# Changfei-Fu/RUMI-SLAM

Hardware: AMD Instinct MI355X
Metric: frames/sec ORB extract+match (higher is better)
Workload: dtype u8; 1 GPU; ORB extract (640x480, 8-level pyramid, 1000 features/frame) + brute-force 256-bit Hamming match of consecutive frames (BASELINE.json configs[1]+[2]); scaling=n/a (one GPU), exchange=none

## Files before the change

include/rumi_testhooks.h:

```cpp
#ifndef RUMI_TESTHOOKS_H
#define RUMI_TESTHOOKS_H
#include <stdint.h>
#ifdef __cplusplus
extern "C" {
#endif

int rumi_hook_sort_like_std(uint32_t *keys, uint16_t *ids, int32_t n);
int rumi_hook_sort_device(uint32_t *keys, uint16_t *ids, int32_t n);
int rumi_hook_std_sort(uint32_t *keys, uint16_t *ids, int32_t n);

int rumi_hook_quadtree(const uint32_t *cand, int32_t n, int32_t minX, int32_t maxX, int32_t minY, int32_t maxY,
                       int32_t N, int32_t *out_idx, int32_t cap, int32_t *n_out);

float rumi_hook_sinf(float x);
float rumi_hook_cosf(float x);
float rumi_hook_fast_atan2(float y, float x);
int rumi_hook_cv_round(float v);
int rumi_hook_magic_div(int32_t idx, int32_t d);

int rumi_hook_lane_packing(int32_t w, int32_t h, float scale, int32_t nlevels, int32_t nframes, int32_t kernel, int32_t level, int32_t force_g,
                           int32_t *info, int32_t *slots, int32_t cap, int32_t *n_out);

struct RumiMatcher;
int rumi_hook_newpts_matches(struct RumiMatcher *m, int32_t n_neigh, int32_t n1, int32_t *matches);

#ifdef __cplusplus
}
#endif
#endif
```

rumi_slam_amd/capi.py:

```python
import ctypes as C
import os

import numpy as np

_HERE = os.path.dirname(os.path.abspath(__file__))
LIB_PATH = os.path.join(_HERE, "librumi_hip.so")

RUMI_OK, RUMI_E_INVALID, RUMI_E_NO_DEVICE, RUMI_E_CAPACITY, RUMI_E_EMPTY = 0, -1, -2, -3, -4

KP_DTYPE = np.dtype([("x", "<f4"), ("y", "<f4"), ("size", "<f4"), ("angle", "<f4"),
                     ("response", "<f4"), ("octave", "<i4"), ("class_id", "<i4")])
assert KP_DTYPE.itemsize == 28


class RumiOrbConfig(C.Structure):
    _fields_ = [("nfeatures", C.c_int32), ("scale_factor", C.c_float), ("nlevels", C.c_int32),
                ("ini_th_fast", C.c_int32), ("min_th_fast", C.c_int32), ("max_width", C.c_int32),
                ("max_height", C.c_int32), ("max_batch", C.c_int32), ("device", C.c_int32),
                ("host_threads", C.c_int32), ("blur_variant", C.c_int32)]


class RumiStreamFrame(C.Structure):
    _fields_ = [("n", C.c_int32), ("mono", C.c_int32), ("n_prev", C.c_int32), ("kp", C.c_void_p), ("desc", C.c_void_p),
                ("best_idx", C.c_void_p), ("best_dist", C.c_void_p), ("second_dist", C.c_void_p)]
# ... 40 lines not shown
    L.rumi_orb_extract_batch_device_async.argtypes = L.rumi_orb_extract_batch_device.argtypes
    L.rumi_orb_sync.argtypes = [vp]
    L.rumi_orb_extract_batch_records_async.argtypes = [vp, vp, i32, i32, i32, i32, i64, i32, i32, vp, i64, i32, vp]
    L.rumi_orb_extract_batch_host.argtypes = [vp, vp, i32, i32, i32, i32, i32, i32, vp, vp, vp, i32, vp, vp, vp, vp]
    L.rumi_orb_extract_batch_host_records.argtypes = [vp, vp, i32, i32, i32, i32, i32, i32, vp, i64, i32, vp, vp]
    L.rumi_orb_pyramid_level.argtypes = [vp, i32, i32, i32, i32, vp, i32, C.POINTER(i32), C.POINTER(i32)]
    L.rumi_orb_stage_keypoints.argtypes = [vp, i32, i32, i32, vp, i32, C.POINTER(i32)]
    L.rumi_orb_set_profiling.argtypes = [vp, i32]
    L.rumi_orb_set_resident_queue.argtypes = [vp, i32]
    L.rumi_orb_wait_event.argtypes = [vp, vp]
    L.rumi_orb_stage_ms.argtypes = [vp, vp]
    L.rumi_orb_stream_create.argtypes = [vp, C.POINTER(vp)]
    L.rumi_orb_stream_destroy.argtypes = [vp]
    L.rumi_orb_stream_destroy.restype = None
    L.rumi_orb_stream_reset.argtypes = [vp]
    L.rumi_orb_stream_push.argtypes = [vp, vp, i32, i32, i32, i32, i32, C.POINTER(RumiStreamFrame)]
    L.rumi_orb_stream_resident.argtypes = [vp, C.POINTER(vp), C.POINTER(vp), C.POINTER(vp)]
    _lib = L
    return L


def check(code):
    if code != RUMI_OK:
        raise RumiError(code, lib().rumi_last_error().decode("utf-8", "replace"))


def ptr(a):
    return a.ctypes.data_as(C.c_void_p)


MATCH_SYMBOLS = ["rumi_descriptor_distance", "rumi_match_create", "rumi_match_destroy", "rumi_search_by_projection_mappoints",
                 "rumi_search_by_projection_frame", "rumi_search_by_bow", "rumi_search_by_bow_kf", "rumi_search_by_projection_sim3",
                 "rumi_search_by_projection_reloc", "rumi_search_for_initialization", "rumi_search_for_triangulation", "rumi_fuse_candidates", "rumi_search_by_sim3", "rumi_frame_is_in_frustum", "rumi_search_local_points", "rumi_search_by_bow_batch", "rumi_match_bruteforce_batch_device", "rumi_match_bruteforce_batch_device_strided", "rumi_match_bruteforce_ring_device", "rumi_match_bruteforce_shape", "rumi_submap_match",
                 "rumi_match_bruteforce_pair_scratch_bytes", "rumi_match_bruteforce_pair_shape", "rumi_match_bruteforce_pair_device"]

OPT_SYMBOLS = ["rumi_opt_create", "rumi_opt_destroy", "rumi_pose_optimization", "rumi_pose_optimization_batch", "rumi_local_ba", "rumi_local_ba_batch", "rumi_merge_ba", "rumi_bundle_adjustment", "rumi_sim3_inliers",
               "rumi_optimize_sim3", "rumi_sim3_ransac", "rumi_opt_stage_ms", "rumi_opt_set_profiling", "rumi_opt_kernel_ms",
               "rumi_essential_graph", "rumi_sim3_correct_points"]

VOC_SYMBOLS = ["rumi_voc_create", "rumi_voc_load_text", "rumi_voc_destroy", "rumi_voc_words", "rumi_voc_levels", "rumi_voc_set_levels", "rumi_voc_assemble", "rumi_voc_transform_features",
               "rumi_voc_transform_batch_device", "rumi_voc_transform"]
TRACK_SYMBOLS = ["rumi_track_create", "rumi_track_destroy", "rumi_track_frame", "rumi_track_extract", "rumi_track_motion",
                 "rumi_track_reference_keyframe", "rumi_track_local", "rumi_track_image_buffer", "rumi_track_last_projections", "rumi_track_set_distortion", "rumi_track_undistorted"]
QUEUE_SYMBOLS = ["rumi_queue_create", "rumi_queue_destroy", "rumi_queue_shards", "rumi_queue_record_bytes", "rumi_queue_block_capacity", "rumi_queue_row",
                 "rumi_queue_uses_rccl", "rumi_queue_extract", "rumi_queue_last_ms"]
KFDB_SYMBOLS = ["rumi_kfdb_create", "rumi_kfdb_destroy", "rumi_kfdb_clear", "rumi_kfdb_size", "rumi_kfdb_next_seq", "rumi_kfdb_max_batch", "rumi_kfdb_add",
                "rumi_kfdb_add_batch_device", "rumi_kfdb_bow", "rumi_kfdb_erase", "rumi_kfdb_clear_map", "rumi_kfdb_set_map_bad", "rumi_kfdb_set_maps",
                "rumi_kfdb_set_bad", "rumi_kfdb_set_covisibles", "rumi_kfdb_score", "rumi_kfdb_scored", "rumi_kfdb_select_reloc", "rumi_kfdb_select_nbest"]
MAPPING_SYMBOLS = ["rumi_create_new_map_points", "rumi_refresh_create", "rumi_refresh_destroy", "rumi_refresh_map_points", "rumi_refresh_stage_ms",
                   "rumi_cull_create", "rumi_cull_destroy", "rumi_keyframe_culling", "rumi_cull_stage_ms"]


def kfdb_lib():
    L = lib()
    if getattr(L, "_kfdb_ready", False):
        return L
    vp, i32, i64, u64 = C.c_void_p, C.c_int32, C.c_int64, C.c_uint64
    L.rumi_kfdb_create.argtypes = [vp, i32, i64, i32, C.POINTER(vp)]
    L.rumi_kfdb_destroy.argtypes = [vp]
    L.rumi_kfdb_destroy.restype = None
    L.rumi_kfdb_clear.argtypes = [vp]
    L.rumi_kfdb_size.argtypes = [vp]
    L.rumi_kfdb_next_seq.argtypes = [vp]
    L.rumi_kfdb_next_seq.restype = i64
    L.rumi_kfdb_max_batch.argtypes = [vp]
    L.rumi_kfdb_add.argtypes = [vp, i32, vp, vp, vp, vp, vp]
    L.rumi_kfdb_add_batch_device.argtypes = [vp, i32, vp, vp, vp, vp, vp, i32, vp]
    L.rumi_kfdb_bow.argtypes = [vp, u64, vp, vp, i32, C.POINTER(i32)]
    L.rumi_kfdb_erase.argtypes = [vp, i32, vp]
    L.rumi_kfdb_clear_map.argtypes = [vp, i32]
    L.rumi_kfdb_set_map_bad.argtypes = [vp, i32, i32]
    L.rumi_kfdb_set_maps.argtypes = [vp, i32, vp, vp]
    L.rumi_kfdb_set_bad.argtypes = [vp, i32, vp, vp]
    L.rumi_kfdb_set_covisibles.argtypes = [vp, i32, vp, vp]
    L.rumi_kfdb_score.argtypes = [vp, i32, i32, vp, vp, vp, vp, vp, vp, vp, vp, vp]
    L.rumi_kfdb_scored.argtypes = [vp, vp, vp]
    L.rumi_kfdb_select_reloc.argtypes = [vp, vp, vp, i64]
    L.rumi_kfdb_select_nbest.argtypes = [vp, vp, i32, vp, vp, vp, vp]
    L._kfdb_ready = True
    return L


HOOK_SYMBOLS = ["rumi_hook_sort_like_std", "rumi_hook_sort_device", "rumi_hook_std_sort", "rumi_hook_quadtree", "rumi_hook_sinf", "rumi_hook_cosf",
                "rumi_hook_fast_atan2", "rumi_hook_cv_round", "rumi_hook_magic_div", "rumi_hook_newpts_matches", "rumi_hook_lane_packing"]


def hooks():
    L = lib()
    if getattr(L, "_hooks_ready", False):
        return L
    vp, i32 = C.c_void_p, C.c_int32
    L.rumi_hook_sort_like_std.argtypes = [vp, vp, i32]
    L.rumi_hook_sort_device.argtypes = [vp, vp, i32]
    L.rumi_hook_std_sort.argtypes = [vp, vp, i32]
    L.rumi_hook_quadtree.argtypes = [vp, i32, i32, i32, i32, i32, i32, vp, i32, C.POINTER(i32)]
    for name in ("rumi_hook_sinf", "rumi_hook_cosf"):
        getattr(L, name).restype = C.c_float
        getattr(L, name).argtypes = [C.c_float]
    L.rumi_hook_fast_atan2.restype = C.c_float
    L.rumi_hook_fast_atan2.argtypes = [C.c_float, C.c_float]
    L.rumi_hook_cv_round.argtypes = [C.c_float]
    L.rumi_hook_magic_div.argtypes = [i32, i32]
    L.rumi_hook_lane_packing.argtypes = [i32, i32, C.c_float, i32, i32, i32, i32, i32, vp, vp, i32, C.POINTER(i32)]
    L._hooks_ready = True
    return L
```

rumi_slam_amd/csrc/orb_kernels.hip:

```cpp
#include <hip/hip_runtime.h>

#include "orb_device.h"
#include "orb_math.h"

namespace rumi {

struct PatternF { float v[256 * 4]; };
constexpr PatternF make_pattern_f() {
    constexpr int8_t src[256 * 4] = {
#include "orb_pattern.inc"
    };
    PatternF p{};
    for (int i = 0; i < 256 * 4; i++) p.v[i] = (float)src[i];
    return p;
}
__constant__ PatternF c_patternF = make_pattern_f();

__device__ __forceinline__ unsigned xcd_swizzle(unsigned lin, unsigned total) {
    const unsigned q = total >> 3, r = total & 7, xcd = lin & 7;
    return (xcd < r ? xcd * (q + 1) : r * (q + 1) + (xcd - r) * q) + (lin >> 3);
}

struct __attribute__((packed)) U32 { uint32_t v; };
struct __attribute__((packed)) U64 { uint64_t v; };
// ... 744 lines not shown
        C = *reinterpret_cast<const uint32_t *>(row);
        H = 0;
        if (!kPacked && haloOff) H = *reinterpret_cast<const uint32_t *>(row + haloOff);
    };
#pragma unroll
    for (int j = 0; j < 7; j++) fetch(y0 - 3 + j, Cn[j], Hn[j]);
    uint32_t Cm[7], Hm[7];
    auto walk7 = [&](const uint32_t (&Cc)[7], const uint32_t (&Hc)[7], int r0) {
#pragma unroll
        for (int j = 0; j < 7; j++) {
            const int r = r0 + j;
            if (r >= rEnd) break;
            orow += L.pitch;
            uint32_t C = Cc[j];
            if (edgeWave) {
                const uint32_t c1 = __shfl_up(C, 1), c2 = __shfl_up(c1, 1);
                C = __builtin_amdgcn_perm(C, __builtin_amdgcn_perm(c1, c2, selA), selB);
            }
            uint32_t Lw = __shfl_up(C, 1), Rw = __shfl_down(C, 1);
            if constexpr (kPacked) {
                if (seamWave && first) Lw = __builtin_amdgcn_perm(C, C, 0x01020300u);
            } else {
                if (lane == 0) Lw = firstBlock ? __builtin_amdgcn_perm(C, C, 0x01020300u) : Hc[j];
                if (lane == 63 && !edgeWave && bw == 256) Rw = Hc[j];
            }
            constexpr uint32_t tA = 18u | (34u << 8) | (kT2 << 16) | (kT3 << 24), tB = kT2 | (34u << 8) | (18u << 16);
            const uint32_t A0 = __builtin_amdgcn_alignbyte(C, Lw, 1), A1 = __builtin_amdgcn_alignbyte(C, Lw, 2), A2 = __builtin_amdgcn_alignbyte(C, Lw, 3);
            const uint32_t B0 = __builtin_amdgcn_alignbyte(Rw, C, 1), B1 = __builtin_amdgcn_alignbyte(Rw, C, 2), B2 = __builtin_amdgcn_alignbyte(Rw, C, 3);
            ring[j][0] = (int)__builtin_amdgcn_udot4(B0, tB, __builtin_amdgcn_udot4(A0, tA, 0u, false), false);
            ring[j][1] = (int)__builtin_amdgcn_udot4(B1, tB, __builtin_amdgcn_udot4(A1, tA, 0u, false), false);
            ring[j][2] = (int)__builtin_amdgcn_udot4(B2, tB, __builtin_amdgcn_udot4(A2, tA, 0u, false), false);
            ring[j][3] = (int)__builtin_amdgcn_udot4(Rw, tB, __builtin_amdgcn_udot4(C, tA, 0u, false), false);
            const int y = r - 3;
            if (y >= y0 && produce) {
                uint32_t o[4];
#pragma unroll
                for (int i = 0; i < 4; i++) {
                    uint32_t acc = mad_u24(kT3, (uint32_t)ring[(j + 4) % 7][i], 32768u);
                    acc = mad_u24(kT2, (uint32_t)(ring[(j + 3) % 7][i] + ring[(j + 5) % 7][i]), acc);
                    acc = mad_u24(34u, (uint32_t)(ring[(j + 2) % 7][i] + ring[(j + 6) % 7][i]), acc);
                    acc = mad_u24(18u, (uint32_t)(ring[(j + 1) % 7][i] + ring[j][i]), acc);
                    if (VARIANT) acc = min(acc, 0x00FFFFFFu);
                    o[i] = acc;
                }
                const uint32_t p01 = __builtin_amdgcn_perm(o[1], o[0], 0x0c0c0602u), p23 = __builtin_amdgcn_perm(o[3], o[2], 0x06020c0cu);
                *reinterpret_cast<uint32_t *>(orow) = p01 | p23;
            }
        }
    };
    for (int r0 = y0 - 3; r0 < rEnd; r0 += 7) {
#pragma unroll
        for (int j = 0; j < 7; j++) Cm[j] = Cn[j], Hm[j] = Hn[j];
        if (r0 + 7 < rEnd) {
#pragma unroll
            for (int j = 0; j < 7; j++) fetch(r0 + 7 + j, Cn[j], Hn[j]);
        }
        walk7(Cm, Hm, r0);
    }
}
template <int VARIANT, int kBlurRows>
__global__ __launch_bounds__(256) void k_blur(const DevParams *__restrict__ P, ImgSrc src, BlurGrid G) {
    blur_body<VARIANT, kBlurRows, false>(P, src, G, blockIdx.x, gridDim.x);
}
template <int VARIANT>
__global__ __launch_bounds__(256) void k_blur_packed(const DevParams *__restrict__ P, ImgSrc src, BlurPack G) {
    blur_body<VARIANT, kBlurRowsBatch, true>(P, src, G, blockIdx.x, gridDim.x);
}
template <int TPC, int VARIANT>
__global__ __launch_bounds__(256) void k_fast_blur(const DevParams *__restrict__ P, ImgSrc src, FastLds F, uint32_t *__restrict__ cellBuf,
                                                   int32_t *__restrict__ cellCnt, BlurGrid G, unsigned gxFast) {
    if (blockIdx.x < gxFast) fast_cells_body<TPC>(P, src, F, cellBuf, cellCnt, blockIdx.x, gxFast);
    else blur_body<VARIANT, kBlurRowsSmall, false>(P, src, G, blockIdx.x - gxFast, gridDim.x - gxFast);
}

__device__ __forceinline__ int half_wave_sum(int v) {
    v += __builtin_amdgcn_update_dpp(0, v, 0x111, 0xF, 0xF, false);
    v += __builtin_amdgcn_update_dpp(0, v, 0x112, 0xF, 0xF, false);
    v += __builtin_amdgcn_update_dpp(0, v, 0x114, 0xF, 0xF, false);
    v += __builtin_amdgcn_update_dpp(0, v, 0x118, 0xF, 0xF, false);
    v += __builtin_amdgcn_update_dpp(0, v, 0x142, 0xA, 0xF, false);
    const int lo = __builtin_amdgcn_readlane(v, 31), hi = __builtin_amdgcn_readlane(v, 63);
    return (threadIdx.x & 32) ? hi : lo;
}
__device__ __forceinline__ int wave_sum(int v) {
#pragma unroll
    for (int o = 32; o > 0; o >>= 1) v += __shfl_xor(v, o);
    return v;
}

constexpr int kDiscP = 48, kPatchP = 48;
constexpr int kKpPerWg = 8;

struct AssembleArgs {
    const uint32_t *selLevel; const int32_t *selLevelCnt; int selLevelCap, lap0, lap1;
    int32_t *counts; long long countsStride; int32_t *errFlag, *errMirror;
    uint32_t *selPackedOut, *selMetaOut; int32_t *selCountOut;
};
template <int kKpGroups, bool kAssemble>
__global__ __launch_bounds__(256, 7) void k_orient_desc(const DevParams *__restrict__ P, ImgSrc src,
                                                     const uint32_t *__restrict__ selPacked,
                                                     const uint32_t *__restrict__ selMeta,
                                                     const int32_t *__restrict__ selCount, int selCap,
                                                     RumiKeyPoint *__restrict__ kpOut, long long kpStride, uint8_t *__restrict__ descOut,
                                                     long long descStride, int outCap, AssembleArgs A) {
    static_assert(kDiscP == kPatchP, "the disc and the patch share their rows");
    __shared__ __attribute__((aligned(16))) uint8_t sWin[kKpPerWg][37 * kPatchP];
    __shared__ __attribute__((aligned(16))) float sPat[256 * 4];
    __shared__ int4 sLv[kMaxLevels];
    __shared__ float2 sLvF[kMaxLevels];
    reinterpret_cast<float4 *>(sPat)[threadIdx.x] = reinterpret_cast<const float4 *>(c_patternF.v)[threadIdx.x];
    if (threadIdx.x < (unsigned)P->nlevels) {
        const DevLevel &Lv = P->lv[threadIdx.x];
        sLv[threadIdx.x] = threadIdx.x == 0 ? make_int4(0, src.l0Pitch, (int)Lv.off, Lv.pitch) : make_int4((int)Lv.off, Lv.pitch, (int)Lv.off, Lv.pitch);
        sLvF[threadIdx.x] = make_float2(Lv.scale, Lv.patchSize);
    }
    const int lane = threadIdx.x & 31, hw = threadIdx.x >> 5;
    const unsigned wg = xcd_swizzle(blockIdx.y * gridDim.x + blockIdx.x, gridDim.x * gridDim.y);
    const int kb = (wg % gridDim.x) * (kKpPerWg * kKpGroups) + hw, frame = wg / gridDim.x;
    int cnt;
    __shared__ uint32_t sOwnPk[kAssemble ? kKpPerWg * kKpGroups : 1], sOwnMt[kAssemble ? kKpPerWg * kKpGroups : 1];
    if constexpr (!kAssemble) {
        cnt = selCount[frame];
        __syncthreads();
    } else {
        __shared__ int sLvStart[kMaxLevels + 1], sRed[2], sOwnF[kKpPerWg * kKpGroups];
        const int nl = P->nlevels, tid = threadIdx.x;
        if (tid == 0) {
            int run = 0;
            for (int l = 0; l < nl; l++) { sLvStart[l] = run; run += A.selLevelCnt[(long long)frame * nl + l]; }
            sLvStart[nl] = run; sRed[0] = 0; sRed[1] = 0;
        }
        __syncthreads();
        const int total = sLvStart[nl], kbase = (wg % gridDim.x) * (kKpPerWg * kKpGroups);
        const bool first = wg % gridDim.x == 0, over = total > selCap;
        int32_t *counts = reinterpret_cast<int32_t *>(reinterpret_cast<uint8_t *>(A.counts) + frame * A.countsStride);
        if (over) {
            if (first && tid == 0) { A.selCountOut[frame] = 0; counts[0] = total; counts[1] = 0; const int old = atomicOr(A.errFlag, 8); if (A.errMirror) *A.errMirror = old | 8; }
            return;
        }
        cnt = total;
        auto key_at = [&](int k, int *levelOut) -> uint32_t {
            int level = 0;
            while (k >= sLvStart[level + 1]) level++;
            *levelOut = level;
            return A.selLevel[((long long)frame * nl + level) * A.selLevelCap + (k - sLvStart[level])];
        };
        auto lapped = [&](uint32_t pk, int level) -> bool {
            float x = (float)((int)(pk & 0xFFF) + kBorder);
            if (level != 0) x = x * P->lv[level].scale;
            return x >= (float)A.lap0 && x <= (float)A.lap1;
        };
        int before = 0, all = 0;
        for (int k = tid; k < total; k += 256) {
            int level;
            const uint32_t pk = key_at(k, &level);
            const int f = lapped(pk, level) ? 1 : 0;
            all += f; before += k < kbase ? f : 0;
        }
#pragma unroll
        for (int o = 32; o > 0; o >>= 1) { before += __shfl_xor(before, o); all += __shfl_xor(all, o); }
        if ((tid & 63) == 0) { atomicAdd(&sRed[0], before); atomicAdd(&sRed[1], all); }
        if (tid < kKpPerWg * kKpGroups) {
            const int k = kbase + tid;
            int level = 0;
            uint32_t pk = 0;
            int f = 0;
            if (k < total) { pk = key_at(k, &level); f = lapped(pk, level) ? 1 : 0; }
            sOwnPk[tid] = pk; sOwnMt[tid] = (uint32_t)level; sOwnF[tid] = f;
        }
        __syncthreads();
        if (tid == 0) {
            int b = sRed[0];
            for (int j = 0; j < kKpPerWg * kKpGroups; j++) {
                const int k = kbase + j;
                if (k >= total) break;
                const int f = sOwnF[j], slot = f ? (total - 1 - b) : (k - b);
                b += f;
                sOwnMt[j] |= (uint32_t)slot << 8;
            }
            if (first) {
                counts[0] = total; counts[1] = total - sRed[1];
                A.selCountOut[frame] = total;
                if (A.errMirror) *A.errMirror = *A.errFlag;
            }
        }
        __syncthreads();
        if (tid < kKpPerWg * kKpGroups && kbase + tid < total) {
            A.selPackedOut[(long long)frame * selCap + kbase + tid] = sOwnPk[tid];
            A.selMetaOut[(long long)frame * selCap + kbase + tid] = sOwnMt[tid];
        }
    }
#ifdef RUMI_OD_STAMP
    long long st[8] = {0, 0, 0, 0, 0, 0, 0, 0}, stLast = clock64();
#define OD_STAMP(k) do { const long long t_ = clock64(); st[k] += t_ - stLast; stLast = t_; } while (0)
#else
#define OD_STAMP(k) do { } while (0)
#endif

    struct __attribute__((packed, aligned(4))) Q16 { uint32_t x, y, z, w; };
    struct __attribute__((packed, aligned(4))) Q8 { uint32_t x, y; };
    auto ld16 = [](const uint8_t *q) { const Q16 t = *reinterpret_cast<const Q16 *>(q); return make_uint4(t.x, t.y, t.z, t.w); };
    auto ld8 = [](const uint8_t *q) { const Q8 t = *reinterpret_cast<const Q8 *>(q); return make_uint2(t.x, t.y); };
    struct Staged { uint4 d0, d1, p0, p1, q0, q1; uint2 p2, q2; uint32_t d2; };
    const bool dRow = lane < 31, qRow = lane < 5;
    const uint8_t *frame0 = src.l0 + (long long)frame * src.l0FrameStride, *framePyr = src.pyr + (long long)frame * P->arenaStride,
                  *frameBlur = src.blur + (long long)frame * P->arenaStride;
    auto fetch_disc = [&](uint32_t pk, uint32_t meta, bool live, Staged &S) {
        if (!live || !dRow) return;
        const int level = meta & 0xFF, x = (int)(pk & 0xFFF) + kBorder, y = (int)((pk >> 12) & 0xFFF) + kBorder;
        const int4 lv = sLv[level];
        const uint8_t *cr = (level == 0 ? frame0 : framePyr) + (lv.x + (y - kHalfPatch + lane) * lv.y + ((x - kHalfPatch) & ~3));
        S.d0 = ld16(cr); S.d1 = ld16(cr + 16); S.d2 = *reinterpret_cast<const uint32_t *>(cr + 32);
    };
    auto fetch_patch = [&](uint32_t pk, uint32_t meta, bool live, Staged &S) {
        if (!live) return;
        const int level = meta & 0xFF, x = (int)(pk & 0xFFF) + kBorder, y = (int)((pk >> 12) & 0xFFF) + kBorder;
        const int4 lv = sLv[level];
        const uint8_t *br = frameBlur + (lv.z + (y - 18 + lane) * lv.w + ((x - 18) & ~3)), *br2 = br + 32 * lv.w;
        S.p0 = ld16(br); S.p1 = ld16(br + 16); S.p2 = ld8(br + 32);
        if (qRow) { S.q0 = ld16(br2); S.q1 = ld16(br2 + 16); S.q2 = ld8(br2 + 32); }
    };
    auto stage_disc = [&](bool live, const Staged &S) {
        if (!live || !dRow) return;
        uint8_t *dst = &sWin[hw][lane * kDiscP];
        *reinterpret_cast<uint4 *>(dst) = S.d0; *reinterpret_cast<uint4 *>(dst + 16) = S.d1; *reinterpret_cast<uint32_t *>(dst + 32) = S.d2;
    };
    auto stage_patch = [&](bool live, const Staged &S) {
        if (!live) return;
        {
            uint8_t *dst = &sWin[hw][lane * kPatchP];
            *reinterpret_cast<uint4 *>(dst) = S.p0; *reinterpret_cast<uint4 *>(dst + 16) = S.p1; *reinterpret_cast<uint2 *>(dst + 32) = S.p2;
        }
        if (qRow) {
            uint8_t *dst = &sWin[hw][(lane + 32) * kPatchP];
            *reinterpret_cast<uint4 *>(dst) = S.q0; *reinterpret_cast<uint4 *>(dst + 16) = S.q1; *reinterpret_cast<uint2 *>(dst + 32) = S.q2;
        }
    };
    auto orientation = [&](uint32_t pk) -> float {
        const int x = (int)(pk & 0xFFF) + kBorder;
        const int xd = (x - kHalfPatch) & ~3;
        const uint8_t *dc = &sWin[hw][kHalfPatch * kDiscP + (x - xd)];
        const int u = lane - kHalfPatch;
        const int vmaxU = lane < 31 ? P->umax[u < 0 ? -u : u] : -1;
        const int mid = dc[u];
        int colSum = vmaxU >= 0 ? mid : 0, m01 = 0;
#pragma unroll
        for (int v = 1; v <= kHalfPatch; v++) {
            const int lo = dc[-v * kDiscP + u], hi = dc[v * kDiscP + u];
            const bool in = v <= vmaxU;
            colSum += in ? lo + hi : 0;
            m01 += in ? v * (hi - lo) : 0;
        }
        int m10 = u * colSum;
        m10 = half_wave_sum(m10);
        m01 = half_wave_sum(m01);
        OD_STAMP(4);
        return fast_atan2_deg((float)m01, (float)m10);
    };
    auto describe = [&](uint32_t pk, uint32_t meta, float angle) {
        const int level = meta & 0xFF, slot = (int)(meta >> 8);
        const int x = (int)(pk & 0xFFF) + kBorder, y = (int)((pk >> 12) & 0xFFF) + kBorder, score = (int)(pk >> 24);
        const int xp = (x - 18) & ~3;
        const float factorPI = (float)(3.1415926535897932384626433832795 / 180.f);
        const float ang = angle * factorPI;
        const float a = cosf_glibc(ang), b = sinf_glibc(ang);
        const uint8_t *bc = &sWin[hw][18 * kPatchP + (x - xp)];
        uint32_t w = 0;
        OD_STAMP(5);
#pragma unroll
        for (int j = 0; j < 8; j++) {
            const float4 pt = reinterpret_cast<const float4 *>(sPat)[j * 32 + lane];
            const float x0 = pt.x, y0 = pt.y, x1 = pt.z, y1 = pt.w;
            const int r0 = cv_round_f(x0 * b + y0 * a), c0 = cv_round_f(x0 * a - y0 * b);
            const int r1 = cv_round_f(x1 * b + y1 * a), c1 = cv_round_f(x1 * a - y1 * b);
            const int t0 = bc[r0 * kPatchP + c0], t1 = bc[r1 * kPatchP + c1];
            const unsigned long long bal = __ballot(t0 < t1);
            const uint32_t lo = (uint32_t)bal, hi = (uint32_t)(bal >> 32);
            asm("s_nop 4\n\tv_writelane_b32 %0, %1, %3\n\tv_writelane_b32 %0, %2, %4" : "+v"(w) : "s"(lo), "s"(hi), "n"(j), "n"(32 + j));
        }
        OD_STAMP(6);
        if (slot < outCap) {
            if (lane < 8) reinterpret_cast<uint32_t *>(descOut + frame * descStride + (long long)slot * 32)[lane] = w;
            if (lane == 0) {
                RumiKeyPoint kp;
                kp.x = (float)x; kp.y = (float)y;
                const float2 lf = sLvF[level];
                if (level != 0) { kp.x = kp.x * lf.x; kp.y = kp.y * lf.x; }
                kp.size = lf.y;
                kp.angle = angle;
                kp.response = (float)score;
                kp.octave = level;
                kp.class_id = -1;
                reinterpret_cast<RumiKeyPoint *>(reinterpret_cast<uint8_t *>(kpOut) + frame * kpStride)[slot] = kp;
            }
        }
    };

    const uint32_t *selP = selPacked + (long long)frame * selCap, *selM = selMeta + (long long)frame * selCap;
    auto key_rec = [&](int k, uint32_t &pk, uint32_t &mt) {
        if constexpr (kAssemble) { const int j = k - (kb - hw); pk = sOwnPk[j]; mt = sOwnMt[j]; }
        else { pk = selP[k]; mt = selM[k]; }
    };
    bool liveC = kb < cnt, liveN = kb + kKpPerWg < cnt;
    uint32_t pkC = 0, mtC = 0, pkN = 0, mtN = 0;
    if (liveC) key_rec(kb, pkC, mtC);
    if (liveN && kKpGroups > 1) key_rec(kb + kKpPerWg, pkN, mtN);
    if (kKpGroups == 1) liveN = false;
    Staged S;
    fetch_disc(pkC, mtC, liveC, S);
    fetch_patch(pkC, mtC, liveC, S);
#pragma unroll
    for (int g = 0; g < kKpGroups; g++) {
        if (!__any(liveC)) break;
        OD_STAMP(0);
        stage_disc(liveC, S);
        OD_STAMP(1);
        const int k2 = kb + (g + 2) * kKpPerWg;
        const bool liveNN = g + 2 < kKpGroups && k2 < cnt;
        uint32_t pkNN = 0, mtNN = 0;
        if (liveNN) key_rec(k2, pkNN, mtNN);
        if (g + 1 < kKpGroups) fetch_disc(pkN, mtN, liveN, S);
        OD_STAMP(2);
        float angle = 0.f;
        if (liveC) angle = orientation(pkC);
        stage_patch(liveC, S);
        if (g + 1 < kKpGroups) fetch_patch(pkN, mtN, liveN, S);
        if (liveC) describe(pkC, mtC, angle);
        OD_STAMP(3);
        pkC = pkN; mtC = mtN; liveC = liveN;
        pkN = pkNN; mtN = mtNN; liveN = liveNN;
    }
#ifdef RUMI_OD_STAMP
    if (threadIdx.x == 0 && (blockIdx.x % 8) == 0 && blockIdx.y == 0) printf("od wg %d: loop-head %lld stage(wait loads) %lld issue-next %lld | IC_Angle %lld trig %lld rBRIEF %lld store %lld\n", (int)blockIdx.x, st[0], st[1], st[2], st[4], st[5], st[6], st[3]);
#endif
}

static long long pack_span(const DevParams &hP, const ImgSrc &src, bool readsLevel0) {
    if (readsLevel0 && src.l0FrameStride <= 0) return 0;
    return readsLevel0 ? std::max(hP.arenaStride, src.l0FrameStride) : hP.arenaStride;
}
void launch_resize(const DevParams *dP, const DevParams &hP, ImgSrc src, const int16_t *coef, const RowTap *rowTab, int level, int nframes,
                   hipStream_t st, int32_t *clearWord) {
    const int rows = hP.lv[level].h >= 200 ? 8 : 4;
    const LanePack K = resize_pack_of(hP.lv[level].w, nframes, pack_span(hP, src, level == 1));
    dim3 g(K.waves, (hP.lv[level].h + 4 * rows - 1) / (4 * rows), (nframes + K.G - 1) / K.G);
    if (rows == 8) hipLaunchKernelGGL(k_resize<8>, g, dim3(256), 0, st, dP, src, coef, rowTab, level, clearWord, K, nframes);
    else hipLaunchKernelGGL(k_resize<4>, g, dim3(256), 0, st, dP, src, coef, rowTab, level, clearWord, K, nframes);
}
void launch_pyramid_tiles(const DevParams *dP, ImgSrc src, const int16_t *coef, const RowTap *rowTab, const PyrTile *tiles, int ntiles, int bufBytes,
                          int tabEntries, int nframes, hipStream_t st, int32_t *clearWord) {
    hipLaunchKernelGGL(k_pyramid_tiles, dim3(ntiles, nframes), dim3(256), (size_t)2 * bufBytes + (size_t)tabEntries * 8, st, dP, src, coef, rowTab, tiles, bufBytes, clearWord);
}
static FastLds fast_lds_of(const DevParams &hP) {
    int wMax = 0, hMax = 0;
    for (int l = 0; l < hP.nlevels; l++) { wMax = std::max(wMax, hP.lv[l].wCell); hMax = std::max(hMax, hP.lv[l].hCell); }
    FastLds F;
    F.tp = 4 * (((wMax + 3) >> 2) + 2);
    F.sp = F.tp;
    F.tileBytes = (hMax + 6) * F.tp;
    F.scBytes = ((hMax + 2) * F.sp + 15) & ~15;
    F.maxIters = (wMax * hMax + 63) / 64 + 1;
    F.tileBytes = (F.tileBytes + 15) & ~15;
    F.perWave = (F.tileBytes + F.scBytes + std::max(kRingCap * 2, F.maxIters * 8) + kScoredCap * 2 + 15) & ~15;
    return F;
}
void launch_fast(const DevParams *dP, const DevParams &hP, ImgSrc src, uint32_t *cellBuf, int32_t *cellCnt, int nframes,
                 hipStream_t st) {
    const FastLds F = fast_lds_of(hP);
    const int wpg = 4;
    const dim3 grid((hP.totalCells + wpg - 1) / wpg, nframes);
    const size_t lds = (size_t)wpg * F.perWave;
#define RUMI_FAST_CASE(T)                                                                                      \
    if (F.tp == T) {                                                                                           \
        hipLaunchKernelGGL((k_fast_cells<T>), grid, dim3(64 * wpg), lds, st, dP, src, F, cellBuf, cellCnt);    \
        return;                                                                                                \
    }
    RUMI_FAST_CASE(48) RUMI_FAST_CASE(44) RUMI_FAST_CASE(52) RUMI_FAST_CASE(56)
#undef RUMI_FAST_CASE
    hipLaunchKernelGGL((k_fast_cells<0>), grid, dim3(64 * wpg), lds, st, dP, src, F, cellBuf, cellCnt);
}
static int compactSlices(int nframes) { return nframes < 32 ? 32 : 8; }
void launch_compact(const DevParams *dP, const DevParams &hP, const uint32_t *cellBuf, const int32_t *cellCnt,
                    uint32_t *cand, int32_t *levelStart, int32_t *errFlag, int nframes, hipStream_t st) {
    hipLaunchKernelGGL(k_compact, dim3(nframes, compactSlices(nframes)), dim3(kCompactThreads), (hP.totalCells + 1) * sizeof(int), st, dP, cellBuf, cellCnt,
                       cand, levelStart, errFlag);
}
static int blur_strip_width(int w) {
    for (int bw : {256, 240, 224, 208}) {
        const int r = w % bw;
        const bool partialInFirstLanes = r >= 1 && r <= 8;
        const bool lane63Halo = bw == 256 && (r >= 253 || r <= 3);
        if (!partialInFirstLanes && !lane63Halo) return bw;
    }
    return 192;
}
static BlurGrid blur_grid_of(const DevParams &hP, int rows, int *total) {
    BlurGrid G{};
    int run = 0;
    for (int l = 0; l < hP.nlevels; l++) {
        G.bw[l] = blur_strip_width(hP.lv[l].w);
        G.gx[l] = (hP.lv[l].w + G.bw[l] - 1) / G.bw[l];
        G.base[l] = run;
        run += G.gx[l] * ((hP.lv[l].h + 4 * rows - 1) / (4 * rows));
    }
    G.base[hP.nlevels] = run;
    *total = run;
    return G;
}
bool fast_blur_fusable(const DevParams &hP) { return fast_lds_of(hP).tp == 48; }
bool launch_fast_blur(const DevParams *dP, const DevParams &hP, ImgSrc src, uint32_t *cellBuf, int32_t *cellCnt, int nframes, int variant, hipStream_t st) {
    const FastLds F = fast_lds_of(hP);
    if (F.tp != 48) return false;
    int run = 0;
    const BlurGrid G = blur_grid_of(hP, kBlurRowsSmall, &run);
    const int wpg = 4;
    const unsigned gxFast = (unsigned)((hP.totalCells + wpg - 1) / wpg);
// ... 59 lines not shown
```

rumi_slam_amd/csrc/orb_math.h:

```cpp
#pragma once
#include <cfloat>
#include <cstdint>
#include <cstring>

#if defined(__HIPCC__)
#define RUMI_HD __host__ __device__ inline
#else
#define RUMI_HD inline
#endif

namespace rumi {

RUMI_HD int cv_round_f(float v) { return (int)__builtin_rintf(v); }

RUMI_HD float fast_atan2_deg(float y, float x) {
    const float kRad2Deg = (float)(180 / 3.1415926535897932384626433832795);
    const float p1 = 0.9997878412794807f * kRad2Deg;
    const float p3 = -0.3258083974640975f * kRad2Deg;
    const float p5 = 0.1555786518463281f * kRad2Deg;
    const float p7 = -0.04432655554792128f * kRad2Deg;
    const float ax = __builtin_fabsf(x), ay = __builtin_fabsf(y);
    float a, c, c2;
    if (ax >= ay) {
        c = ay / (ax + (float)DBL_EPSILON);
        c2 = c * c;
        a = (((p7 * c2 + p5) * c2 + p3) * c2 + p1) * c;
    } else {
        c = ax / (ay + (float)DBL_EPSILON);
        c2 = c * c;
        a = 90.f - (((p7 * c2 + p5) * c2 + p3) * c2 + p1) * c;
    }
    if (x < 0) a = 180.f - a;
    if (y < 0) a = 360.f - a;
    return a;
}

namespace sincosf_impl {
struct Tab { double c0, c1, c2, c3, c4, s1, s2, s3; };
RUMI_HD float poly(double x, double x2, bool negCos, int n) {
    const double sg = negCos ? -1.0 : 1.0;
    const double c0 = sg * 0x1p0, c1 = sg * -0x1.ffffffd0c621cp-2, c2c = sg * 0x1.55553e1068f19p-5,
                 c3 = sg * -0x1.6c087e89a359dp-10, c4 = sg * 0x1.99343027bf8c3p-16;
    const double s1c = -0x1.555545995a603p-3, s2c = 0x1.1107605230bc4p-7, s3c = -0x1.994eb3774cf24p-13;
    if ((n & 1) == 0) {
        double x3 = x * x2;
        double s1 = s2c + x2 * s3c;
        double x7 = x3 * x2;
        double s = x + x3 * s1c;
        return (float)(s + x7 * s1);
    } else {
        double x4 = x2 * x2;
        double cc2 = c3 + x2 * c4;
        double cc1 = c0 + x2 * c1;
        double x6 = x4 * x2;
        double c = cc1 + x4 * c2c;
        return (float)(c + x6 * cc2);
    }
}
RUMI_HD uint32_t top12(float f) {
    uint32_t u;
#if defined(__HIP_DEVICE_COMPILE__)
    u = __float_as_uint(f);
#else
    std::memcpy(&u, &f, 4);
#endif
    return (u >> 20) & 0x7ff;
}
RUMI_HD float eval(float y, int isCos) {
    double x = y;
    if (top12(y) < top12(0x1.921FB6p-1f)) {
        if (top12(y) < top12(0x1p-12f)) return isCos ? 1.0f : y;
        return poly(x, x * x, false, isCos);
    }
    const double r = x * 0x1.45F306DC9C883p+23;
    const int n = ((int32_t)r + 0x800000) >> 24;
    x = x - n * 0x1.921FB54442D18p0;
    const double s = ((n & 3) == 1 || (n & 3) == 2) ? -1.0 : 1.0;
    return poly(x * s, x * x, (n & 2) != 0, n ^ isCos);
}
}
RUMI_HD float sinf_glibc(float x) { return sincosf_impl::eval(x, 0); }
RUMI_HD float cosf_glibc(float x) { return sincosf_impl::eval(x, 1); }

}
```

rumi_slam_amd/csrc/testhooks.hip:

```cpp
#include <hip/hip_runtime.h>

#include <vector>

#include "orb_geom.h"
#include "orb_math.h"
#include "orb_octree.h"
#include "rumi_orb.h"
#include <algorithm>
#include <utility>
#include <vector>

#include "rumi_testhooks.h"

using namespace rumi;

extern "C" int rumi_hook_sort_like_std(uint32_t *keys, uint16_t *ids, int32_t n) {
    if (n < 0 || (n > 0 && (!keys || !ids))) return RUMI_E_INVALID;
    std::vector<OctEntry> e((size_t)n);
    for (int i = 0; i < n; i++) e[i] = OctEntry{keys[i], ids[i], 0};
    sort_like_libstdcxx(e.data(), n);
    for (int i = 0; i < n; i++) { keys[i] = e[i].key; ids[i] = e[i].id; }
    return RUMI_OK;
}

namespace rumi { int launch_sort_hook(uint32_t *keys, uint16_t *ids, int n); }
extern "C" int rumi_hook_sort_device(uint32_t *keys, uint16_t *ids, int32_t n) { return rumi::launch_sort_hook(keys, ids, n); }
extern "C" int rumi_hook_std_sort(uint32_t *keys, uint16_t *ids, int32_t n) {
    if (n < 0) return -1;
    std::vector<std::pair<uint32_t, uint16_t>> v(n);
    for (int i = 0; i < n; i++) v[i] = {keys[i], ids[i]};
    std::sort(v.begin(), v.end(), [](const std::pair<uint32_t, uint16_t> &a, const std::pair<uint32_t, uint16_t> &b) { return a.first < b.first; });
    for (int i = 0; i < n; i++) { keys[i] = v[i].first; ids[i] = v[i].second; }
    return 0;
}

extern "C" int rumi_hook_quadtree(const uint32_t *cand, int32_t n, int32_t minX, int32_t maxX, int32_t minY,
                                  int32_t maxY, int32_t N, int32_t *out_idx, int32_t cap, int32_t *n_out) {
    if (!n_out || n < 0 || n > 65535 || maxX <= minX || maxY <= minY) return RUMI_E_INVALID;
    std::vector<int> out;
    int m = octree_host(cand, n, minX, maxX, minY, maxY, N, out);
    if (m < 0) return RUMI_E_INVALID;
    *n_out = m;
    if (m > cap) return RUMI_E_CAPACITY;
    for (int i = 0; i < m; i++) out_idx[i] = out[i];
    return RUMI_OK;
}

extern "C" float rumi_hook_sinf(float x) { return sinf_glibc(x); }
extern "C" float rumi_hook_cosf(float x) { return cosf_glibc(x); }
extern "C" float rumi_hook_fast_atan2(float y, float x) { return fast_atan2_deg(y, x); }
extern "C" int rumi_hook_cv_round(float v) { return cv_round_f(v); }
extern "C" int rumi_hook_magic_div(int32_t idx, int32_t d) { return magic_div(idx, magic_of((unsigned)d)); }

extern "C" int rumi_hook_lane_packing(int32_t w, int32_t h, float scale, int32_t nlevels, int32_t nframes, int32_t kernel, int32_t level,
                                      int32_t force_g, int32_t *info, int32_t *slots, int32_t cap, int32_t *n_out) {
    if (!info || !n_out || nframes < 1 || nlevels < 1 || nlevels > kMaxLevels || kernel < 0 || kernel > 1 || level < (kernel ? 0 : 1) || level >= nlevels ||
        force_g < 0 || force_g > nframes)
        return RUMI_E_INVALID;
    const OrbTables t = make_tables(1000, scale, nlevels);
    std::vector<LevelGeom> g;
    long long arena = 0;
    int cells, cand, cellCand;
    if (!make_geometry(t, w, h, g, &arena, &cells, &cand, &cellCand)) return RUMI_E_INVALID;
    const long long span = std::max(arena, (long long)w * h);
    LanePack K = kernel ? blur_pack_of(g[level].w, nframes, span) : resize_pack_of(g[level].w, nframes, span);
    if (force_g) { K.G = force_g; K.waves = lane_pack_waves(K.lpr, K.G, K.step); }
    const int groups = (nframes + K.G - 1) / K.G;
    const int32_t inf[8] = {g[level].w, K.lpr, K.G, K.waves, groups, K.step, K.halo, g[level].h};
    std::copy(inf, inf + 8, info);
    const long long n = (long long)groups * K.waves * 64;
    *n_out = (int32_t)std::min<long long>(n, INT32_MAX);
    if (n > cap || !slots) return RUMI_E_CAPACITY;
    int32_t *o = slots;
    for (int grp = 0; grp < groups; grp++)
        for (int wv = 0; wv < K.waves; wv++)
            for (int lane = 0; lane < 64; lane++, o += 3) {
                const LaneSlot s = lane_slot(K, wv, lane);
                const int f = lane_frame(K, s, grp, nframes);
                o[0] = f; o[1] = s.col; o[2] = (f >= 0 && s.produce ? 1 : 0) | (s.first ? 2 : 0) | (s.last ? 4 : 0);
            }
    return RUMI_OK;
}
```

Before: 313,200 frames/s.

## Compute IC_Angle moments in registers with udot4 and share steering trig across key-points

Orientation moments are now computed per disc row directly from the registers holding that row, using byte-align plus udot4 with a precomputed umax row mask. This removes the LDS staging of the disc and the column-wise LDS reads. With two key-point groups, both discs are fetched up front and a single fast_atan2/sin/cos pass serves both key-points, with odd lanes working on the second one and results broadcast by DPP. The per-group loop is replaced by straight-line code. The trade-off is higher register pressure from keeping two discs live (the code adds an explicit VGPR clobber), plus a new host test hook that checks the moment math.

```diff
diff --git a/include/rumi_testhooks.h b/include/rumi_testhooks.h
--- a/include/rumi_testhooks.h
+++ b/include/rumi_testhooks.h
@@ -16,6 +16,7 @@
 float rumi_hook_cosf(float x);
 float rumi_hook_fast_atan2(float y, float x);
 int rumi_hook_cv_round(float v);
+int rumi_hook_disc_row_moments(const uint8_t *row36, int32_t a, int32_t umax_v, int32_t v, int32_t *m10, int32_t *m01);
 int rumi_hook_magic_div(int32_t idx, int32_t d);
 
 int rumi_hook_lane_packing(int32_t w, int32_t h, float scale, int32_t nlevels, int32_t nframes, int32_t kernel, int32_t level, int32_t force_g,
diff --git a/rumi_slam_amd/capi.py b/rumi_slam_amd/capi.py
--- a/rumi_slam_amd/capi.py
+++ b/rumi_slam_amd/capi.py
@@ -146,7 +146,7 @@
 
 
 HOOK_SYMBOLS = ["rumi_hook_sort_like_std", "rumi_hook_sort_device", "rumi_hook_std_sort", "rumi_hook_quadtree", "rumi_hook_sinf", "rumi_hook_cosf",
-                "rumi_hook_fast_atan2", "rumi_hook_cv_round", "rumi_hook_magic_div", "rumi_hook_newpts_matches", "rumi_hook_lane_packing"]
+                "rumi_hook_fast_atan2", "rumi_hook_cv_round", "rumi_hook_disc_row_moments", "rumi_hook_magic_div", "rumi_hook_newpts_matches", "rumi_hook_lane_packing"]
 
 
 def hooks():
@@ -164,6 +164,7 @@
     L.rumi_hook_fast_atan2.restype = C.c_float
     L.rumi_hook_fast_atan2.argtypes = [C.c_float, C.c_float]
     L.rumi_hook_cv_round.argtypes = [C.c_float]
+    L.rumi_hook_disc_row_moments.argtypes = [vp, i32, i32, i32, C.POINTER(i32), C.POINTER(i32)]
     L.rumi_hook_magic_div.argtypes = [i32, i32]
     L.rumi_hook_lane_packing.argtypes = [i32, i32, C.c_float, i32, i32, i32, i32, i32, vp, vp, i32, C.POINTER(i32)]
     L._hooks_ready = True
diff --git a/rumi_slam_amd/csrc/orb_kernels.hip b/rumi_slam_amd/csrc/orb_kernels.hip
--- a/rumi_slam_amd/csrc/orb_kernels.hip
+++ b/rumi_slam_amd/csrc/orb_kernels.hip
@@ -850,13 +850,17 @@
     const int lo = __builtin_amdgcn_readlane(v, 31), hi = __builtin_amdgcn_readlane(v, 63);
     return (threadIdx.x & 32) ? hi : lo;
 }
+template <int kCtrl>
+__device__ __forceinline__ float quad_bcast(float v) {
+    return __int_as_float(__builtin_amdgcn_update_dpp(0, __float_as_int(v), kCtrl, 0xF, 0xF, false));
+}
 __device__ __forceinline__ int wave_sum(int v) {
 #pragma unroll
     for (int o = 32; o > 0; o >>= 1) v += __shfl_xor(v, o);
     return v;
 }
 
-constexpr int kDiscP = 48, kPatchP = 48;
+constexpr int kPatchP = 48;
 constexpr int kKpPerWg = 8;
 
 struct AssembleArgs {
@@ -871,7 +875,6 @@
                                                      const int32_t *__restrict__ selCount, int selCap,
                                                      RumiKeyPoint *__restrict__ kpOut, long long kpStride, uint8_t *__restrict__ descOut,
                                                      long long descStride, int outCap, AssembleArgs A) {
-    static_assert(kDiscP == kPatchP, "the disc and the patch share their rows");
     __shared__ __attribute__((aligned(16))) uint8_t sWin[kKpPerWg][37 * kPatchP];
     __shared__ __attribute__((aligned(16))) float sPat[256 * 4];
     __shared__ int4 sLv[kMaxLevels];
@@ -969,18 +972,19 @@
     struct __attribute__((packed, aligned(4))) Q8 { uint32_t x, y; };
     auto ld16 = [](const uint8_t *q) { const Q16 t = *reinterpret_cast<const Q16 *>(q); return make_uint4(t.x, t.y, t.z, t.w); };
     auto ld8 = [](const uint8_t *q) { const Q8 t = *reinterpret_cast<const Q8 *>(q); return make_uint2(t.x, t.y); };
-    struct Staged { uint4 d0, d1, p0, p1, q0, q1; uint2 p2, q2; uint32_t d2; };
+    struct Disc { uint4 d0, d1; uint32_t d2; };
+    struct Patch { uint4 p0, p1, q0, q1; uint2 p2, q2; };
     const bool dRow = lane < 31, qRow = lane < 5;
     const uint8_t *frame0 = src.l0 + (long long)frame * src.l0FrameStride, *framePyr = src.pyr + (long long)frame * P->arenaStride,
                   *frameBlur = src.blur + (long long)frame * P->arenaStride;
-    auto fetch_disc = [&](uint32_t pk, uint32_t meta, bool live, Staged &S) {
+    auto fetch_disc = [&](uint32_t pk, uint32_t meta, bool live, Disc &D) {
         if (!live || !dRow) return;
         const int level = meta & 0xFF, x = (int)(pk & 0xFFF) + kBorder, y = (int)((pk >> 12) & 0xFFF) + kBorder;
         const int4 lv = sLv[level];
         const uint8_t *cr = (level == 0 ? frame0 : framePyr) + (lv.x + (y - kHalfPatch + lane) * lv.y + ((x - kHalfPatch) & ~3));
-        S.d0 = ld16(cr); S.d1 = ld16(cr + 16); S.d2 = *reinterpret_cast<const uint32_t *>(cr + 32);
+        D.d0 = ld16(cr); D.d1 = ld16(cr + 16); D.d2 = *reinterpret_cast<const uint32_t *>(cr + 32);
     };
-    auto fetch_patch = [&](uint32_t pk, uint32_t meta, bool live, Staged &S) {
+    auto fetch_patch = [&](uint32_t pk, uint32_t meta, bool live, Patch &S) {
         if (!live) return;
         const int level = meta & 0xFF, x = (int)(pk & 0xFFF) + kBorder, y = (int)((pk >> 12) & 0xFFF) + kBorder;
         const int4 lv = sLv[level];
@@ -988,12 +992,7 @@
         S.p0 = ld16(br); S.p1 = ld16(br + 16); S.p2 = ld8(br + 32);
         if (qRow) { S.q0 = ld16(br2); S.q1 = ld16(br2 + 16); S.q2 = ld8(br2 + 32); }
     };
-    auto stage_disc = [&](bool live, const Staged &S) {
-        if (!live || !dRow) return;
-        uint8_t *dst = &sWin[hw][lane * kDiscP];
-        *reinterpret_cast<uint4 *>(dst) = S.d0; *reinterpret_cast<uint4 *>(dst + 16) = S.d1; *reinterpret_cast<uint32_t *>(dst + 32) = S.d2;
-    };
-    auto stage_patch = [&](bool live, const Staged &S) {
+    auto stage_patch = [&](bool live, const Patch &S) {
         if (!live) return;
         {
             uint8_t *dst = &sWin[hw][lane * kPatchP];
@@ -1004,37 +1003,34 @@
             *reinterpret_cast<uint4 *>(dst) = S.q0; *reinterpret_cast<uint4 *>(dst + 16) = S.q1; *reinterpret_cast<uint2 *>(dst + 32) = S.q2;
         }
     };
-    auto orientation = [&](uint32_t pk) -> float {
+    uint32_t rowMask[8];
+    {
+        const int v = lane - kHalfPatch;
+        disc_row_mask(dRow ? P->umax[v < 0 ? -v : v] : -1, rowMask);
+    }
+    auto moments = [&](uint32_t pk, bool live, const Disc &D, int &m01, int &m10) {
         const int x = (int)(pk & 0xFFF) + kBorder;
-        const int xd = (x - kHalfPatch) & ~3;
-        const uint8_t *dc = &sWin[hw][kHalfPatch * kDiscP + (x - xd)];
-        const int u = lane - kHalfPatch;
-        const int vmaxU = lane < 31 ? P->umax[u < 0 ? -u : u] : -1;
-        const int mid = dc[u];
-        int colSum = vmaxU >= 0 ? mid : 0, m01 = 0;
-#pragma unroll
-        for (int v = 1; v <= kHalfPatch; v++) {
-            const int lo = dc[-v * kDiscP + u], hi = dc[v * kDiscP + u];
-            const bool in = v <= vmaxU;
-            colSum += in ? lo + hi : 0;
-            m01 += in ? v * (hi - lo) : 0;
-        }
-        int m10 = u * colSum;
-        m10 = half_wave_sum(m10);
-        m01 = half_wave_sum(m01);
-        OD_STAMP(4);
-        return fast_atan2_deg((float)m01, (float)m10);
+        const uint32_t d[9] = {D.d0.x, D.d0.y, D.d0.z, D.d0.w, D.d1.x, D.d1.y, D.d1.z, D.d1.w, D.d2};
+        int r10, r01;
+        disc_row_moments(d, (x - kHalfPatch) & 3, rowMask, lane - kHalfPatch, &r10, &r01);
+        r10 = half_wave_sum(r10);
+        r01 = half_wave_sum(r01);
+        m10 = live ? r10 : 0; m01 = live ? r01 : 0;
     };
-    auto describe = [&](uint32_t pk, uint32_t meta, float angle) {
+    struct Steer { float angle, a, b; };
+    auto steer = [&](int m01, int m10) -> Steer {
+        const float factorPI = (float)(3.1415926535897932384626433832795 / 180.f);
+        const float angle = fast_atan2_deg((float)m01, (float)m10);
+        const float ang = angle * factorPI;
+        return Steer{angle, cosf_glibc(ang), sinf_glibc(ang)};
+    };
+    auto describe = [&](uint32_t pk, uint32_t meta, const Steer &T) {
         const int level = meta & 0xFF, slot = (int)(meta >> 8);
         const int x = (int)(pk & 0xFFF) + kBorder, y = (int)((pk >> 12) & 0xFFF) + kBorder, score = (int)(pk >> 24);
         const int xp = (x - 18) & ~3;
-        const float factorPI = (float)(3.1415926535897932384626433832795 / 180.f);
-        const float ang = angle * factorPI;
-        const float a = cosf_glibc(ang), b = sinf_glibc(ang);
+        const float angle = T.angle, a = T.a, b = T.b;
         const uint8_t *bc = &sWin[hw][18 * kPatchP + (x - xp)];
         uint32_t w = 0;
-        OD_STAMP(5);
 #pragma unroll
         for (int j = 0; j < 8; j++) {
             const float4 pt = reinterpret_cast<const float4 *>(sPat)[j * 32 + lane];
@@ -1069,37 +1065,44 @@
         if constexpr (kAssemble) { const int j = k - (kb - hw); pk = sOwnPk[j]; mt = sOwnMt[j]; }
         else { pk = selP[k]; mt = selM[k]; }
     };
-    bool liveC = kb < cnt, liveN = kb + kKpPerWg < cnt;
+    static_assert(kKpGroups == 1 || kKpGroups == 2, "one key-point per half wave, or two with one steering pass for both");
+    if constexpr (kKpGroups == 2) asm volatile("" ::: "v64");
+    const bool liveC = kb < cnt, liveN = kKpGroups > 1 && kb + kKpPerWg < cnt;
     uint32_t pkC = 0, mtC = 0, pkN = 0, mtN = 0;
     if (liveC) key_rec(kb, pkC, mtC);
-    if (liveN && kKpGroups > 1) key_rec(kb + kKpPerWg, pkN, mtN);
-    if (kKpGroups == 1) liveN = false;
-    Staged S;
-    fetch_disc(pkC, mtC, liveC, S);
-    fetch_patch(pkC, mtC, liveC, S);
-#pragma unroll
-    for (int g = 0; g < kKpGroups; g++) {
-        if (!__any(liveC)) break;
-        OD_STAMP(0);
-        stage_disc(liveC, S);
-        OD_STAMP(1);
-        const int k2 = kb + (g + 2) * kKpPerWg;
-        const bool liveNN = g + 2 < kKpGroups && k2 < cnt;
-        uint32_t pkNN = 0, mtNN = 0;
-        if (liveNN) key_rec(k2, pkNN, mtNN);
-        if (g + 1 < kKpGroups) fetch_disc(pkN, mtN, liveN, S);
-        OD_STAMP(2);
-        float angle = 0.f;
-        if (liveC) angle = orientation(pkC);
-        stage_patch(liveC, S);
-        if (g + 1 < kKpGroups) fetch_patch(pkN, mtN, liveN, S);
-        if (liveC) describe(pkC, mtC, angle);
+    if (liveN) key_rec(kb + kKpPerWg, pkN, mtN);
+    Disc DC = {}, DN = {};
+    Patch Pt;
+    fetch_disc(pkC, mtC, liveC, DC);
+    if (kKpGroups > 1) fetch_disc(pkN, mtN, liveN, DN);
+    fetch_patch(pkC, mtC, liveC, Pt);
+    if (!__any(liveC)) return;
+    OD_STAMP(0);
+    int m01C, m10C, m01N = 0, m10N = 0;
+    moments(pkC, liveC, DC, m01C, m10C);
+    if (kKpGroups > 1) moments(pkN, liveN, DN, m01N, m10N);
+    OD_STAMP(4);
+    Steer tC, tN = {0.f, 0.f, 0.f};
+    if constexpr (kKpGroups == 1) {
+        tC = steer(m01C, m10C);
+    } else {
+        const bool odd = lane & 1;
+        const Steer t = steer(odd ? m01N : m01C, odd ? m10N : m10C);
+        tC = Steer{quad_bcast<0x00>(t.angle), quad_bcast<0x00>(t.a), quad_bcast<0x00>(t.b)};
+        tN = Steer{quad_bcast<0x55>(t.angle), quad_bcast<0x55>(t.a), quad_bcast<0x55>(t.b)};
+    }
+    OD_STAMP(5);
+    stage_patch(liveC, Pt);
+    if (kKpGroups > 1) fetch_patch(pkN, mtN, liveN, Pt);
+    if (liveC) describe(pkC, mtC, tC);
+    OD_STAMP(3);
+    if constexpr (kKpGroups > 1) {
+        stage_patch(liveN, Pt);
+        if (liveN) describe(pkN, mtN, tN);
         OD_STAMP(3);
-        pkC = pkN; mtC = mtN; liveC = liveN;
-        pkN = pkNN; mtN = mtNN; liveN = liveNN;
     }
 #ifdef RUMI_OD_STAMP
-    if (threadIdx.x == 0 && (blockIdx.x % 8) == 0 && blockIdx.y == 0) printf("od wg %d: loop-head %lld stage(wait loads) %lld issue-next %lld | IC_Angle %lld trig %lld rBRIEF %lld store %lld\n", (int)blockIdx.x, st[0], st[1], st[2], st[4], st[5], st[6], st[3]);
+    if (threadIdx.x == 0 && (blockIdx.x % 8) == 0 && blockIdx.y == 0) printf("od wg %d: issue loads %lld | wait + IC_Angle %lld trig %lld stage + rBRIEF %lld store %lld\n", (int)blockIdx.x, st[0], st[4], st[5], st[6], st[3]);
 #endif
 }
 
diff --git a/rumi_slam_amd/csrc/orb_math.h b/rumi_slam_amd/csrc/orb_math.h
--- a/rumi_slam_amd/csrc/orb_math.h
+++ b/rumi_slam_amd/csrc/orb_math.h
@@ -33,6 +33,38 @@
     if (x < 0) a = 180.f - a;
     if (y < 0) a = 360.f - a;
     return a;
+}
+
+RUMI_HD void disc_row_mask(int um, uint32_t mask[8]) {
+    const uint32_t bits = um < 0 ? 0u : ((2u << (2 * um)) - 1u) << (15 - um);
+    for (int k = 0; k < 8; k++) {
+        const uint32_t ones = (((bits >> (4 * k)) & 0xFu) * 0x00204081u) & 0x01010101u;
+        mask[k] = (ones << 8) - ones;
+    }
+}
+RUMI_HD void disc_row_moments(const uint32_t d[9], int a, const uint32_t mask[8], int v, int *m10, int *m01) {
+    uint32_t S = 0, T = 0;
+#if defined(__HIP_DEVICE_COMPILE__)
+#pragma unroll
+    for (int k = 0; k < 8; k++) {
+        const uint32_t b = __builtin_amdgcn_alignbyte(d[k + 1], d[k], (uint32_t)a) & mask[k];
+        const uint32_t j4 = 0x03020100u + 0x04040404u * (uint32_t)k;
+        S = __builtin_amdgcn_udot4(b, 0x01010101u, S, false);
+        T = __builtin_amdgcn_udot4(b, j4, T, false);
+    }
+#else
+    for (int k = 0; k < 8; k++) {
+        const uint64_t two = ((uint64_t)d[k + 1] << 32) | d[k];
+        const uint32_t b = (uint32_t)(two >> (8 * (a & 3))) & mask[k];
+        for (int i = 0; i < 4; i++) {
+            const uint32_t px = (b >> (8 * i)) & 0xFF;
+            S += px;
+            T += (uint32_t)(4 * k + i) * px;
+        }
+    }
+#endif
+    *m10 = (int)T - 15 * (int)S;
+    *m01 = v * (int)S;
 }
 
 namespace sincosf_impl {
diff --git a/rumi_slam_amd/csrc/testhooks.hip b/rumi_slam_amd/csrc/testhooks.hip
--- a/rumi_slam_amd/csrc/testhooks.hip
+++ b/rumi_slam_amd/csrc/testhooks.hip
@@ -50,6 +50,16 @@
 extern "C" float rumi_hook_cosf(float x) { return cosf_glibc(x); }
 extern "C" float rumi_hook_fast_atan2(float y, float x) { return fast_atan2_deg(y, x); }
 extern "C" int rumi_hook_cv_round(float v) { return cv_round_f(v); }
+extern "C" int rumi_hook_disc_row_moments(const uint8_t *row36, int32_t a, int32_t umax_v, int32_t v, int32_t *m10, int32_t *m01) {
+    if (!row36 || !m10 || !m01 || a < 0 || a > 3 || umax_v > 15 || v < -15 || v > 15) return RUMI_E_INVALID;
+    uint32_t d[9], mask[8];
+    std::memcpy(d, row36, 36);
+    disc_row_mask(umax_v, mask);
+    int s10, s01;
+    disc_row_moments(d, a, mask, v, &s10, &s01);
+    *m10 = s10; *m01 = s01;
+    return RUMI_OK;
+}
 extern "C" int rumi_hook_magic_div(int32_t idx, int32_t d) { return magic_div(idx, magic_of((unsigned)d)); }
 
 extern "C" int rumi_hook_lane_packing(int32_t w, int32_t h, float scale, int32_t nlevels, int32_t nframes, int32_t kernel, int32_t level,
```

Result: no change. 316,100 frames/s, median of 6 (+0.9%).
